# citiususc/BigSeqKit

Hardware: AMD Instinct MI355X
Metric: M records/s + GB/s (vs HBM roofline) on 100GB FASTQ stats (higher is better)
Workload: dtype u8; 1 GPU; bigseqkit stats on 100.0 GB synthetic FASTQ-150 (BASELINE C2: 315457413 records x 317 B), HBM-resident, 1 record-aligned shard(s); command=stats, records=315457413, bytes=99999999921, seed=42

## Files before the change

bigseqkit_amd/_lib.py:

```python
import ctypes as C
import os

_HERE = os.path.dirname(os.path.abspath(__file__))
LIB_PATH = os.environ.get("BSK_LIB", os.path.join(_HERE, "lib", "libbsk.so"))

if not os.path.exists(LIB_PATH):
    raise ImportError(
        f"libbsk.so not found at {LIB_PATH}: build it with ./build.sh "
        "(hipcc --offload-arch=gfx950); bigseqkit_amd has no CPU fallback")



def _preload_hip_runtime():
    import importlib.util
    try:
        spec = importlib.util.find_spec("torch")
    except Exception:
        spec = None
    if spec and spec.origin:
        cand = os.path.join(os.path.dirname(spec.origin), "lib", "libamdhip64.so")
        if os.path.exists(cand):
            try:
                C.CDLL(cand, mode=C.RTLD_GLOBAL)
            except OSError:
# ... 139 lines not shown
    "bsk_event_destroy": (_i, [_vp]),
    "bsk_selftest_regex_find": (_i, [C.c_char_p, C.c_char_p, _sz, _sz, _p(C.c_uint32), _p(C.c_uint32)]),
    "bsk_store_open": (_i, [C.c_char_p, _i, _p(_vp)]),
    "bsk_store_error": (C.c_char_p, [_vp]),
    "bsk_store_put": (_i, [_vp, _vp, _u64, _vp]),
    "bsk_store_put_host": (_i, [_vp, _u64, _vp, _sz]),
    "bsk_store_close": (_i, [_vp, _p(_u64)]),
    "bsk_run_to_store": (_i, [_vp, _vp, _sz, _i, _i64, _vp, _u64, _p(_u64), _p(_u64)]),
    "bsk_profile_enable": (_i, [_vp, _i]),
    "bsk_profile_read": (_i, [_vp, C.c_char_p, _p(C.c_double), _p(_u64)]),
    "bsk_profile_reset": (_i, [_vp]),
    "bsk_profile_dump": (_i, [_vp, C.c_char_p, _sz]),
    "bsk_selftest_scan": (_i, [_i, _p(C.c_uint32), _p(C.c_uint32)]),
    "bsk_selftest_rmdup_keys": (_i, [_vp, _p(_u64), _p(_u64), _sz, _p(_sz)]),
    "bsk_selftest_stream_read": (_i, [_vp, _sz, _i, _i, _p(C.c_float)]),
}

for _name, (_res, _args) in SIGNATURES.items():
    _f = getattr(lib, _name)
    _f.restype = _res
    _f.argtypes = _args


class BskError(RuntimeError):
    def __init__(self, code, message):
        super().__init__(message)
        self.code = code


def check(rc, ctx=None):
# ... 5 lines not shown
```

bigseqkit_amd/csrc/capi.cpp:

```cpp
#include <hip/hip_runtime_api.h>

#include <algorithm>
#include <cstdio>
#include <cstdlib>
#include <cstring>
#include <new>
#include <optional>

#include "../../include/bsk.h"
#include "anchor.hpp"
#include "ctx.hpp"
#include "ops_host.hpp"
#include "ops_host_internal.hpp"
#include "ops_segcopy.hpp"
#include "stats_host.hpp"
#include "stream_stats.hpp"
#include "regex_vm.hpp"
#include "synth.hpp"

namespace bsk {
hipError_t launch_synth(int kind, uint64_t seed, unsigned flags, uint64_t first_record, uint8_t* dst, uint64_t n,
                        hipStream_t st);
}

// ... 288 lines not shown
}

int bsk_rmdup_finish(bsk_ctx* c) {
    if (!c) return BSK_ERR_INVALID_ARG;
    if (c->op != bsk::Op::RmDup) return BSK_OK;
    return bsk::rmdup_finish(c);
}

void bsk_destroy(bsk_ctx* c) {
    if (!c) return;
    if (c->op == bsk::Op::RmDup) bsk::rmdup_finish(c);
    if (c->device >= 0) {
        hipSetDevice(c->device);
        hipDeviceSynchronize();
        for (auto& p : c->pending) { hipEventDestroy(p.a); hipEventDestroy(p.b); }
        bsk::store_drainer_free(c);
        if (c->d_anchors) hipFree(c->d_anchors);
        if (c->d_rng) hipFree(c->d_rng);
        if (c->d_parts) hipFree(c->d_parts);
        if (c->d_vec) hipFree(c->d_vec);
        if (c->d_pack) hipFree(c->d_pack);
        if (c->h_pack) hipHostFree(c->h_pack);
        if (c->d_ctl) hipFree(c->d_ctl);
        if (c->h_ctl) hipHostFree(c->h_ctl);
        if (c->h_head) hipHostFree(c->h_head);
        if (c->d_overflow) hipFree(c->d_overflow);
        for (void* p : {(void*)c->d_text_w, (void*)c->d_lin_off, (void*)c->d_lin, (void*)c->d_codon, (void*)c->d_keys,
                        (void*)c->d_table})
            if (p) hipFree(p);
        if (c->d_names) hipFree(c->d_names);
// ... 74 lines not shown
}

size_t bsk_stats_vector_len(const bsk_ctx* c) { return c ? (size_t)STATS_HDR + c->hist_cap : 0; }

int bsk_stats_reset(bsk_ctx* c, void* stream) {
    if (!c || c->op != Op::Stats) return fail(c, BSK_ERR_INVALID_ARG, "libbsk: not a Stats context");
    if (c->device < 0) return fail(c, BSK_ERR_NO_DEVICE, "libbsk: context was created without a device");
    BSK_ENTER(c);
    hipStream_t st = (hipStream_t)stream;
    HIP_TRY(c, hipMemsetAsync(c->d_vec, 0, ((size_t)STATS_HDR + c->hist_cap) * sizeof(uint64_t), st));
    HIP_TRY(c, hipMemsetAsync(c->d_ctl, 0, bsk_ctx::CTL_WORDS * sizeof(uint64_t), st));
    c->vec_reduced = false;
    return BSK_OK;
}

static int stats_run_device(bsk_ctx* c, const uint8_t* d_buf, size_t n, int format, uint64_t* d_vec, hipStream_t st) {
    const bool fastq = format == BSK_FORMAT_FASTQ;
    const bool all = c->opts.b("All");
    const bool variant = fastq ? c->stats_a_dense : c->tune.is("stats_fasta", "events");
    const int per_cu = stats_max_blocks_per_cu(fastq, all, c->use_dpp, variant);
    const int blocks = std::max(1, c->num_cus * per_cu);
    const uint64_t waves = (uint64_t)blocks * 4;
    const uint64_t nr = pick_nranges(n, waves, c->min_range_bytes, (int)c->tune.num("ranges_per_wave"));
    const uint32_t nranges = (uint32_t)nr;
    uint64_t chunk = (n + nranges - 1) / nranges;
    chunk = (chunk + 15) & ~(uint64_t)15;
    const bool self_anchor = fastq && !all && c->use_dpp && !c->tune.is("stats_prep", "pass");
    uint32_t tickets = nranges, nsplit = nranges;
    if (self_anchor) {
        chunk = (chunk + 63) & ~(uint64_t)63;
        const uint64_t tail = nranges / 16, small = chunk / 4;
        const uint64_t floor_bytes = std::max<uint64_t>(c->min_range_bytes, (uint64_t)c->tune.num("stats_tail", 192 << 10));
        if (tail && small >= floor_bytes && !c->tune.is("stats_tail", "uniform") && (uint64_t)(nranges - tail) * chunk < n) {
            nsplit = (uint32_t)(nranges - tail);
            tickets = nsplit + (uint32_t)((n - (uint64_t)nsplit * chunk + small - 1) / small);
        }
    } else {
        int rc = ensure_ranges(c, nranges);
        if (rc != BSK_OK) return rc;
    }
    const uint64_t need = n / c->hist_cap + 1024;
    if (need > c->overflow_cap) {
        uint64_t* nb = nullptr;
        HIP_TRY(c, hipMalloc((void**)&nb, need * sizeof(uint64_t)));
        if (c->d_overflow) {
            HIP_TRY(c, hipMemcpyAsync(nb, c->d_overflow, c->overflow_cap * sizeof(uint64_t), hipMemcpyDeviceToDevice, st));
            HIP_TRY(c, hipStreamSynchronize(st));
            HIP_TRY(c, hipFree(c->d_overflow));
        }
        c->d_overflow = nb;
        c->overflow_cap = need;
    }
// ... 34 lines not shown
            c->rng_cap = nranges;
        }
        D.r_head = c->d_rng;
        D.r_tail = c->d_rng + nranges;
        D.r_flags = reinterpret_cast<uint32_t*>(c->d_rng + 2 * (size_t)nranges);
        HIP_TRY(c, hipMemsetAsync(c->d_rng, 0, (size_t)nranges * 20, st));
    }
    if (!self_anchor) {
        Timed t(c, "k_prep", st);
        HIP_TRY(c, launch_prep(fastq, d_buf, n, chunk, nranges, anchors, queue, st, !fastq,
                               fastq ? nullptr : c->d_anchors + (size_t)nranges + 2));
    }
    {
        Timed t(c, "k_stats", st);
        HIP_TRY(c, launch_stats(fastq, all, c->use_dpp, blocks, d_buf, n, anchors, tickets, queue, D, st, variant,
                                !fastq ? chunk : 0, self_anchor ? chunk : 0, nsplit));
    }
    if (!fastq) HIP_TRY(c, launch_stats_stitch(nranges, D, st));
    if (all && (int)gap_letters.size() > MAX_GAP_LETTERS) {
        const int rci = build_index(c, d_buf, n, format, st);
        if (rci != BSK_OK) return rci;
        uint32_t set[8] = {0, 0, 0, 0, 0, 0, 0, 0};
        for (char ch : gap_letters) set[(uint8_t)ch >> 5] |= 1u << ((uint8_t)ch & 31u);
        HIP_TRY(c, launch_gap_set_count(d_buf, c->table, set, fastq, D.vec + 2, st));
    }
    return BSK_OK;
}

static int stage_shard(bsk_ctx* c, const void* shard, size_t n, int on_device, hipStream_t st, const uint8_t** d);

int bsk_stats_run(bsk_ctx* c, const void* shard, size_t n, int on_device, int format, int64_t pid, void* d_vec,
// ... 160 lines not shown
    c->type_if_F = alphabet_name(guess_alphabet_less_conservatively(seq.data(), seq.size(), 10000));
    *n_out = m.size();
    if (m.size() > cap || !keys || !vals) {
        if (cap == 0) return BSK_OK;
        return fail(c, BSK_ERR_CAPACITY, "libbsk: output map does not fit the caller's buffers");
    }
    size_t i = 0;
    for (auto& kv : m) {
        keys[i] = kv.first;
        vals[i] = kv.second;
        ++i;
    }
    return BSK_OK;
}

int bsk_stats_collect(bsk_ctx* c, const void* d_vec, int64_t* keys, int64_t* vals, size_t cap, size_t* n_out) {
    if (!c || c->op != Op::Stats) return fail(c, BSK_ERR_INVALID_ARG, "libbsk: not a Stats context");
    if (c->device < 0) return fail(c, BSK_ERR_NO_DEVICE, "libbsk: context was created without a device");
    if (!n_out) return fail(c, BSK_ERR_INVALID_ARG, "libbsk: null n_out");
    BSK_ENTER(c);
    HIP_TRY(c, hipDeviceSynchronize());
    const uint64_t* dv = d_vec ? (const uint64_t*)d_vec : c->d_vec;
    const uint32_t kbins = std::min<uint32_t>(bsk_ctx::PACK_BINS, c->hist_cap);
    const size_t pack_words = 8 + (size_t)STATS_HDR + kbins;
    if (!c->d_pack) HIP_TRY(c, hipMalloc((void**)&c->d_pack, pack_words * sizeof(uint64_t)));
    if (!c->h_pack) HIP_TRY(c, hipHostMalloc((void**)&c->h_pack, pack_words * sizeof(uint64_t), hipHostMallocDefault));
    HIP_TRY(c, launch_stats_pack(dv, c->hist_cap, c->d_status, c->d_pack, kbins, nullptr));
    HIP_TRY(c, hipMemcpyAsync(c->h_pack, c->d_pack, pack_words * sizeof(uint64_t), hipMemcpyDeviceToHost, nullptr));
    HIP_TRY(c, hipStreamSynchronize(nullptr));
    const uint64_t* status = c->h_pack;
    if (status[0]) {
        int code;
        std::string m = describe_kernel_errors(status[0], &code);
        return fail(c, code, m);
    }
    const size_t ext = (size_t)std::min<uint64_t>(status[2], c->hist_cap);
    const size_t len = (size_t)STATS_HDR + ext;
    std::vector<uint64_t> v(c->h_pack + 8, c->h_pack + 8 + std::min<size_t>(len, (size_t)STATS_HDR + kbins));
    if (ext > kbins) {
        v.resize(len);
        HIP_TRY(c, hipMemcpy(v.data() + STATS_HDR + kbins, dv + STATS_HDR + kbins, (ext - kbins) * sizeof(uint64_t), hipMemcpyDeviceToHost));
    }
    std::vector<uint64_t> ov;
    if (status[1]) {
// ... 603 lines not shown
    return BSK_OK;
}
int bsk_event_elapsed_ms(void* start, void* stop, float* ms) {
    HIP_TRY(nullptr, hipEventSynchronize((hipEvent_t)stop));
    HIP_TRY(nullptr, hipEventElapsedTime(ms, (hipEvent_t)start, (hipEvent_t)stop));
    return BSK_OK;
}
int bsk_event_destroy(void* ev) {
    HIP_TRY(nullptr, hipEventDestroy((hipEvent_t)ev));
    return BSK_OK;
}

int bsk_profile_enable(bsk_ctx* c, int on) {
    if (!c) return BSK_ERR_INVALID_ARG;
    c->profile = on != 0;
    return BSK_OK;
}

int bsk_profile_read(bsk_ctx* c, const char* kernel, double* total_ms, uint64_t* launches) {
    if (!c || !kernel) return BSK_ERR_INVALID_ARG;
    if (c->device >= 0) {
        BSK_ENTER(c);
        for (auto& p : c->pending) {
            HIP_TRY(c, hipEventSynchronize(p.b));
            float ms = 0;
            HIP_TRY(c, hipEventElapsedTime(&ms, p.a, p.b));
            auto& pr = c->prof[p.name];
            pr.ms += ms;
            pr.launches += 1;
            hipEventDestroy(p.a);
            hipEventDestroy(p.b);
        }
        c->pending.clear();
    }
    auto it = c->prof.find(kernel);
    if (total_ms) *total_ms = it == c->prof.end() ? 0.0 : it->second.ms;
    if (launches) *launches = it == c->prof.end() ? 0 : it->second.launches;
    return BSK_OK;
}

int bsk_profile_dump(bsk_ctx* c, char* buf, size_t cap) {
    if (!c || !buf || cap == 0) return BSK_ERR_INVALID_ARG;
    double d;
    uint64_t l;
    int rc = bsk_profile_read(c, "", &d, &l);
    if (rc != BSK_OK) return rc;
    std::string out;
// ... 49 lines not shown
        HIP_TRY(nullptr, hipEventRecord(a, nullptr));
        HIP_TRY(nullptr, launch_stream_read(blocks, (const uint8_t*)d_buf, n, chunk, (uint32_t)nr, d, d + 1, nullptr));
        HIP_TRY(nullptr, hipEventRecord(b, nullptr));
        HIP_TRY(nullptr, hipEventSynchronize(b));
        float ms = 0;
        HIP_TRY(nullptr, hipEventElapsedTime(&ms, a, b));
        if (r > 0) total += ms;
    }
    *avg_ms = total / reps;
    hipEventDestroy(a);
    hipEventDestroy(b);
    hipFree(d);
    return BSK_OK;
}

int bsk_selftest_scan(int use_dpp, const uint32_t* in64, uint32_t* out64) {
    uint32_t *d_in = nullptr, *d_out = nullptr;
    HIP_TRY(nullptr, hipMalloc((void**)&d_in, 64 * 4));
    HIP_TRY(nullptr, hipMalloc((void**)&d_out, 64 * 4));
    HIP_TRY(nullptr, hipMemcpy(d_in, in64, 64 * 4, hipMemcpyHostToDevice));
    HIP_TRY(nullptr, launch_scan_selftest(use_dpp != 0, d_in, d_out, nullptr));
    HIP_TRY(nullptr, hipMemcpy(out64, d_out, 64 * 4, hipMemcpyDeviceToHost));
    hipFree(d_in);
    hipFree(d_out);
    return BSK_OK;
}

int bsk_selftest_regex_find(const char* expr, const uint8_t* text, size_t n, size_t from, uint32_t* caps4, uint32_t* ngroups) {
    try {
        const VmProgram P = compile_vm(expr ? expr : "");
// ... 10 lines not shown
```

bigseqkit_amd/csrc/ctx.hpp:

```cpp
#pragma once
#include <hip/hip_runtime_api.h>

#include <algorithm>
#include <array>
#include <atomic>
#include <cstdlib>
#include <cctype>
#include <cstdint>
#include <cstdio>
#include <cstring>
#include <map>
#include <mutex>
#include <string>
#include <vector>

#include "index.hpp"
#include "opts.hpp"
#include "regex_nfa.hpp"
#include "regex_vm.hpp"

struct bsk_tuning {
    static const char* const* names() {
        static const char* const N[] = {"filter", "grep_shiftand", "head_genome_window", "index", "locate_nopre", "long_bytes", "min_range_bytes", "names",
                                        "names_scale", "out", "pin_alphabet", "ranges_per_wave", "replace", "rmdup", "rmdup_buckets", "rmdup_hash", "rmdup_k1_bits", "rmdup_k2_bits", "rmdup_keys", "rmdup_place", "rmdup_xcheck", "rmdup_xlocal", "scan", "segcopy",
                                        "sort", "stage_bytes", "stats_a", "stats_fasta", "stats_prep", "stats_tail", "subseq", "subseq_scale", "text", "translate", "translate_index", "translate_probe", "translate_stream", "tr_lanes", nullptr};
        return N;
    }
    std::map<std::string, std::string> v;
    static bool known(const std::string& k) {
        for (const char* const* n = names(); *n; ++n) if (k == *n) return true;
        return false;
    }
    void load_env() {
        for (const char* const* n = names(); *n; ++n) {
            std::string e = "BSK_";
            for (const char* q = *n; *q; ++q) e.push_back((char)toupper((unsigned char)*q));
            if (const char* val = getenv(e.c_str())) v[*n] = val;
        }
    }
    const char* get(const char* k) const {
// ... 250 lines not shown
    uint64_t slice_src_cap = 0;

    void* drainer = nullptr;
    uint8_t* pinned[2] = {nullptr, nullptr};
    uint8_t* d_stage[2] = {nullptr, nullptr};
    size_t stage_size[2] = {0, 0};
    hipStream_t copy_stream[2] = {nullptr, nullptr};
    hipEvent_t stage_done[2] = {nullptr, nullptr};
    hipEvent_t stage_free[2] = {nullptr, nullptr};

    bool profile = false;
    struct Prof { double ms = 0; uint64_t launches = 0; };
    std::map<std::string, Prof> prof;
    struct PendingEv { const char* name; hipEvent_t a, b; };
    std::vector<PendingEv> pending;

    void set_error(const std::string& m) const {
        std::lock_guard<std::mutex> g(mu);
        last_error = m;
    }

    mutable std::string log_text;
    void log(const char* level, const std::string& m, bool unless_quiet = false) const {
        if (unless_quiet && opts.cb("Quiet")) return;
        const std::string line = std::string("[") + level + "] " + m + "\n";
        {
            std::lock_guard<std::mutex> g(mu);
            log_text += line;
        }
        fputs(line.c_str(), stderr);
// ... 11 lines not shown
        if (owns) ++c->call_gen;
    }
    ~bsk_call_scope() { if (owns) c->busy.store(false, std::memory_order_release); }
    bsk_call_scope(const bsk_call_scope&) = delete;
    bsk_call_scope& operator=(const bsk_call_scope&) = delete;
};
#define BSK_BUSY_TEXT "libbsk: context busy: another call is running on this context (one context per caller thread, include/bsk.h)"

struct Timed {
    bsk_ctx* c;
    const char* name;
    hipStream_t st;
    hipEvent_t a = nullptr, b = nullptr;
    Timed(bsk_ctx* c_, const char* n, hipStream_t s) : c(c_), name(n), st(s) {
        if (c->profile) {
            hipEventCreate(&a);
            hipEventCreate(&b);
            hipEventRecord(a, st);
        }
    }
    ~Timed() {
        if (c->profile && a) {
            hipEventRecord(b, st);
            c->pending.push_back({name, a, b});
        }
    }
};

inline uint64_t pick_nranges(uint64_t n, uint64_t waves, uint64_t min_range_bytes, int pinned = 0) {
    uint64_t nr;
    if (pinned) nr = waves * (uint64_t)pinned;
    else {
        nr = n / (512u * 1024u);
        const uint64_t lo = std::min<uint64_t>(waves * 2, n / (128u * 1024u));
        nr = std::max(nr, lo);
        nr = std::min<uint64_t>(nr, waves * 16);
    }
    nr = std::min<uint64_t>(nr, n / std::max<uint64_t>(1, min_range_bytes));
    return std::max<uint64_t>(1, nr);
// ... 6 lines not shown
```

bigseqkit_amd/csrc/stream_stats.hip:

```cpp
#include <hip/hip_runtime.h>

#include <algorithm>
#include <cstdint>

#include "anchor.hpp"
#include "anchor_wave_dev.hpp"
#include "index.hpp"
#include "stream_core_dev.hpp"
#include "stream_fasta2_dev.hpp"
#include "stream_stats.hpp"

namespace bsk {

namespace {

using namespace stream;

constexpr int BIG_SLOTS = 64;
constexpr uint32_t BIG_EMPTY = 0xFFFFFFFFu;

__device__ __forceinline__ void add_big(uint32_t len, uint32_t c, uint32_t* s_hist, const StatsDev& D) {
    uint32_t* keys = s_hist + LDS_HIST;
    uint32_t* cnts = keys + BIG_SLOTS;
    const uint32_t slot = (len * 2654435761u) >> 26;
// ... 292 lines not shown
#define BSK_STATS_WAVES_FQ 6
#endif
#if BSK_STATS_WAVES
#ifndef BSK_STATS_WAVES_FA_ALL
#define BSK_STATS_WAVES_FA_ALL 5
#endif
#define BSK_STATS_ATTR __attribute__((amdgpu_waves_per_eu((ALL && FASTQ) ? BSK_STATS_WAVES_ALL : (FASTQ ? BSK_STATS_WAVES_FQ : ((ALL && ROLES_T) ? BSK_STATS_WAVES_FA_ALL : BSK_STATS_WAVES)), 8)))
#else
#define BSK_STATS_ATTR
#endif

template <bool FASTQ, bool ALL, bool DPP, bool ROLES_T = true>
__global__ __launch_bounds__(WAVES_PER_BLOCK * WAVE) BSK_STATS_ATTR void k_stats(const uint8_t* __restrict__ buf, uint64_t n,
                                                                   const uint64_t* __restrict__ anchors,
                                                                   uint32_t nranges, uint32_t* __restrict__ queue,
                                                                   StatsDev D, uint64_t chunk, uint32_t nsplit) {
    __shared__ uint32_t s_hist[LDS_HIST + 2 * BIG_SLOTS];
    constexpr bool ROLES = FASTQ && ALL && ROLES_T;
    constexpr bool SALL = ALL && !ROLES;
    constexpr int WINDOW = (FASTQ && !SALL) ? 256 : CAP;
    constexpr bool F2 = !FASTQ && ROLES_T;
    __shared__ Lds<FASTQ, SALL, F2 ? 4 : WINDOW> s_l[F2 ? 1 : WAVES_PER_BLOCK];
    __shared__ LdsF2T<F2 && ALL> s_f2[F2 ? WAVES_PER_BLOCK : 1];
    for (int i = threadIdx.x; i < LDS_HIST + 2 * BIG_SLOTS; i += blockDim.x)
        s_hist[i] = (i >= LDS_HIST && i < LDS_HIST + BIG_SLOTS) ? BIG_EMPTY : 0u;
    __syncthreads();

    const int lane = threadIdx.x & 63;
    const int wave = threadIdx.x >> 6;
    Lds<FASTQ, SALL, F2 ? 4 : WINDOW>& L = s_l[F2 ? 0 : wave];
    StatsSinkT<ROLES> sink;
    sink.s_hist = s_hist;
    sink.D = D;
    constexpr bool SELF = FASTQ && !ALL && DPP;
    const bool self_anchor = SELF && anchors == nullptr;
    const uint64_t n_eff = self_anchor ? wave_anchor::effective_end(buf, n) : anchors[nranges];
    uint64_t w20 = 0, w30 = 0, wgap = 0;
    for (;;) {
        uint32_t r = 0;
        if (lane == 0) r = atomicAdd(queue, 1u);
        r = wave_first(r);
        if (r >= nranges) break;
        uint64_t rs = 0, re = n_eff;
        if (self_anchor) {
            if constexpr (SELF) {
#pragma nounroll
                for (uint32_t k = 0; k < 2u; ++k) {
                    const uint32_t t = r + k;
                    if (t == 0u || t >= nranges) continue;
                    const uint64_t from = t <= nsplit ? (uint64_t)t * chunk : (uint64_t)nsplit * chunk + (uint64_t)(t - nsplit) * (chunk >> 2);
                    uint32_t flo = (uint32_t)from, fhi = (uint32_t)(from >> 32);
                    asm volatile("" : "+v"(flo), "+v"(fhi));
                    const uint64_t av = wave_anchor::fastq_range_start(buf, n, ((uint64_t)fhi << 32) | flo);
                    const uint64_t a = ((uint64_t)wave_first((uint32_t)(av >> 32)) << 32) | wave_first((uint32_t)av);
                    if (k == 0u) rs = a;
                    else re = a;
                }
            }
        } else {
            rs = anchors[r];
            re = anchors[r + 1];
        }
        rs = rs < n_eff ? rs : n_eff;
// ... 168 lines not shown
        const uint64_t rs = (uint64_t)r * chunk, re = (rs + chunk < n) ? rs + chunk : n;
        for (uint64_t t = rs; t < re; t += TILE) {
#pragma unroll
            for (int p = 0; p < NPIECE; ++p) {
                const uint64_t idx = t + (uint64_t)p * PIECE_BYTES + (uint64_t)lane * 16;
                if (idx + 16 <= re) {
                    const uint4 v = *reinterpret_cast<const uint4*>(buf + idx);
                    acc ^= v.x ^ v.y ^ v.z ^ v.w;
                }
            }
        }
    }
    if (acc == 0x9E3779B9u) sink[0] = acc;
}

template <bool DPP>
__global__ void k_scan_selftest(const uint32_t* in, uint32_t* out) {
    out[threadIdx.x] = wave_incl_scan<DPP>(in[threadIdx.x]);
}

}

hipError_t launch_prep(bool fastq, const uint8_t* buf, uint64_t n, uint64_t chunk, uint32_t nranges,
                       uint64_t* anchors, uint32_t* queue, hipStream_t st, bool line_mode, uint64_t* raw) {
    const int threads = 256;
    const int blocks = (int)(((uint64_t)nranges + 1 + 3) / 4);
    if (fastq) hipLaunchKernelGGL(k_prep<true>, dim3(blocks), dim3(threads), 0, st, buf, n, chunk, nranges, anchors, queue, 0);
    else if (line_mode && raw) {
        hipLaunchKernelGGL(k_prep<false>, dim3(blocks), dim3(threads), 0, st, buf, n, chunk, nranges, raw, queue, 2);
        hipLaunchKernelGGL(k_prep_fill, dim3((nranges + 1 + 255) / 256), dim3(256), 0, st, (const uint64_t*)raw, nranges, anchors);
    } else hipLaunchKernelGGL(k_prep<false>, dim3(blocks), dim3(threads), 0, st, buf, n, chunk, nranges, anchors, queue, line_mode ? 1 : 0);
    return hipGetLastError();
}

__global__ __launch_bounds__(1024) void k_stats_pack(const uint64_t* __restrict__ vec, uint32_t cap, const uint64_t* __restrict__ status,
                                                     uint64_t* __restrict__ pack, uint32_t kbins) {
    __shared__ uint32_t s_hi;
    if (threadIdx.x == 0) s_hi = 0;
    __syncthreads();
    const uint64_t* hist = vec + STATS_HDR;
    uint32_t hi = 0;
    for (uint32_t base = threadIdx.x; base < cap; base += 8u * 1024u) {
        uint64_t h[8];
#pragma unroll
        for (uint32_t k = 0; k < 8u; ++k) {
            const uint32_t i = base + k * 1024u;
            h[k] = i < cap ? hist[i] : 0ull;
        }
#pragma unroll
        for (uint32_t k = 0; k < 8u; ++k)
            if (h[k]) hi = base + k * 1024u + 1u;
    }
    if (hi) atomicMax(&s_hi, hi);
    for (uint32_t i = threadIdx.x; i < (uint32_t)STATS_HDR + kbins; i += 1024u) pack[8u + i] = vec[i];
    if (threadIdx.x < 8u && threadIdx.x != 2u) pack[threadIdx.x] = status[threadIdx.x];
    __syncthreads();
    if (threadIdx.x == 0) pack[2] = s_hi;
}

hipError_t launch_stats_pack(const uint64_t* vec, uint32_t cap, const uint64_t* status, uint64_t* pack, uint32_t kbins, hipStream_t st) {
    if (kbins > cap) kbins = cap;
    hipLaunchKernelGGL(k_stats_pack, dim3(1), dim3(1024), 0, st, vec, cap, status, pack, kbins);
    return hipGetLastError();
}

namespace {
struct GapSet { uint32_t w[8]; };
__global__ __launch_bounds__(256) void k_gap_set_count(const uint8_t* __restrict__ buf, RecordTable t, GapSet S, int fastq,
                                                       unsigned long long* __restrict__ gap_slot) {
    const uint32_t lane = threadIdx.x & 63u;
    const uint64_t nwaves = (uint64_t)gridDim.x * (blockDim.x >> 6);
    uint64_t acc = 0;
    for (uint64_t r = (uint64_t)blockIdx.x * (blockDim.x >> 6) + (threadIdx.x >> 6); r < t.n; r += nwaves) {
        const uint64_t from = t.start[r] + t.l_head[r] + 1;
        const uint64_t to = fastq ? from + t.l_seq[r] : t.start[r + 1];
        for (uint64_t i = from + lane; i < to; i += 64) {
            const uint8_t c = buf[i];
// ... 10 lines not shown
    if (t.n == 0) return hipSuccess;
    GapSet S;
    for (int i = 0; i < 8; ++i) S.w[i] = set[i];
    const uint64_t blocks = std::min<uint64_t>((t.n + 3) / 4, 256ull * 32ull);
    hipLaunchKernelGGL(k_gap_set_count, dim3((unsigned)blocks), dim3(256), 0, st, buf, t, S, fastq ? 1 : 0, (unsigned long long*)gap_slot);
    return hipGetLastError();
}

hipError_t launch_stats_stitch(uint32_t nranges, const StatsDev& D, hipStream_t st) {
    hipLaunchKernelGGL(k_stats_stitch, dim3((nranges + 255u) / 256u), dim3(256), 0, st, nranges, D);
    return hipGetLastError();
}

template <bool FASTQ, bool ALL, bool ROLES_T = true>
static hipError_t launch_stats_t(bool dpp, int blocks, const uint8_t* buf, uint64_t n, const uint64_t* anchors,
                                 uint32_t nranges, uint32_t* queue, const StatsDev& D, hipStream_t st, uint64_t chunk, uint32_t nsplit = 0) {
    const dim3 b(WAVES_PER_BLOCK * WAVE);
    if (dpp) hipLaunchKernelGGL((k_stats<FASTQ, ALL, true, ROLES_T>), dim3(blocks), b, 0, st, buf, n, anchors, nranges, queue, D, chunk, nsplit);
    else hipLaunchKernelGGL((k_stats<FASTQ, ALL, false, ROLES_T>), dim3(blocks), b, 0, st, buf, n, anchors, nranges, queue, D, chunk, nsplit);
    return hipGetLastError();
}

hipError_t launch_stats(bool fastq, bool all, bool dpp, int blocks, const uint8_t* buf, uint64_t n,
                        const uint64_t* anchors, uint32_t nranges, uint32_t* queue, const StatsDev& D,
                        hipStream_t st, bool a_dense, uint64_t skip_chunk, uint64_t fq_chunk, uint32_t fq_nsplit) {
    if (fastq && all && a_dense) return launch_stats_t<true, true, false>(dpp, blocks, buf, n, anchors, nranges, queue, D, st, fq_chunk, fq_nsplit);
    if (fastq) return all ? launch_stats_t<true, true>(dpp, blocks, buf, n, anchors, nranges, queue, D, st, fq_chunk, fq_nsplit)
                          : launch_stats_t<true, false>(dpp, blocks, buf, n, anchors, nranges, queue, D, st, fq_chunk, fq_nsplit);
    if (all) return a_dense ? launch_stats_t<false, true, false>(dpp, blocks, buf, n, anchors, nranges, queue, D, st, skip_chunk)
                            : launch_stats_t<false, true>(dpp, blocks, buf, n, anchors, nranges, queue, D, st, skip_chunk);
    return a_dense ? launch_stats_t<false, false, false>(dpp, blocks, buf, n, anchors, nranges, queue, D, st, skip_chunk)
                   : launch_stats_t<false, false>(dpp, blocks, buf, n, anchors, nranges, queue, D, st, skip_chunk);
}

int stats_max_blocks_per_cu(bool fastq, bool all, bool dpp, bool a_dense) {
    int nb = 0;
    const void* f = nullptr;
#define BSK_PICK(FQ, AL, RO)                                                             \
    f = dpp ? (const void*)k_stats<FQ, AL, true, RO> : (const void*)k_stats<FQ, AL, false, RO>;
    if (fastq && all && a_dense) { BSK_PICK(true, true, false) }
    else if (fastq && all) { BSK_PICK(true, true, true) }
    else if (fastq) { BSK_PICK(true, false, true) }
    else if (all && a_dense) { BSK_PICK(false, true, false) }
    else if (all) { BSK_PICK(false, true, true) }
    else if (a_dense) { BSK_PICK(false, false, false) }
    else { BSK_PICK(false, false, true) }
#undef BSK_PICK
    if (hipOccupancyMaxActiveBlocksPerMultiprocessor(&nb, f, WAVES_PER_BLOCK * WAVE, 0) != hipSuccess || nb < 1) nb = 1;
    return nb;
}

hipError_t launch_stream_read(int blocks, const uint8_t* buf, uint64_t n, uint64_t chunk, uint32_t nranges,
                              uint32_t* queue, uint32_t* sink, hipStream_t st) {
    hipLaunchKernelGGL(k_stream_read, dim3(blocks), dim3(WAVES_PER_BLOCK * WAVE), 0, st, buf, n, chunk, nranges, queue,
                       sink);
    return hipGetLastError();
}

hipError_t launch_scan_selftest(bool dpp, const uint32_t* in, uint32_t* out, hipStream_t st) {
    if (dpp) hipLaunchKernelGGL(k_scan_selftest<true>, dim3(1), dim3(64), 0, st, in, out);
    else hipLaunchKernelGGL(k_scan_selftest<false>, dim3(1), dim3(64), 0, st, in, out);
    return hipGetLastError();
}

}
```

bigseqkit_amd/csrc/stream_stats.hpp:

```cpp
#pragma once
#include <hip/hip_runtime_api.h>

#include <cstdint>

namespace bsk {

constexpr int STATS_HDR = 8;
constexpr int MAX_GAP_LETTERS = 8;

constexpr uint32_t ERR_BAD_HEADER = 1u;
constexpr uint32_t ERR_BAD_PLUS = 2u;
constexpr uint32_t ERR_LEN_MISMATCH = 4u;
constexpr uint32_t ERR_TRUNCATED = 8u;
constexpr uint32_t ERR_ANCHOR = 16u;
constexpr uint32_t ERR_LINE_TOO_LONG = 32u;
constexpr uint32_t ERR_CAPACITY = 64u;

struct PredConsts {
    uint32_t k20, k30;
    uint32_t gap_rep[MAX_GAP_LETTERS];
    int ngap;
    uint32_t kgap;
};

// ... 6 lines not shown
    PredConsts pred;
    uint64_t* r_head;
    uint64_t* r_tail;
    uint32_t* r_flags;
};

constexpr uint32_t RF_VISITED = 1u, RF_HAS_HEADER = 2u, RF_HEAD_CLOSED = 4u, RF_TAIL_OPEN = 8u;
constexpr uint32_t RF_MID = 16u, RF_SKIP_SEQ = 32u;

hipError_t launch_prep(bool fastq, const uint8_t* buf, uint64_t n, uint64_t chunk, uint32_t nranges,
                       uint64_t* anchors, uint32_t* queue, hipStream_t st, bool line_mode = false, uint64_t* raw = nullptr);
hipError_t launch_stats_stitch(uint32_t nranges, const StatsDev& D, hipStream_t st);
struct RecordTable;
hipError_t launch_gap_set_count(const uint8_t* buf, const RecordTable& t, const uint32_t (&set)[8], bool fastq, uint64_t* gap_slot,
                                hipStream_t st);
hipError_t launch_stats_pack(const uint64_t* vec, uint32_t cap, const uint64_t* status, uint64_t* pack, uint32_t kbins, hipStream_t st);
hipError_t launch_stats(bool fastq, bool all, bool dpp, int blocks, const uint8_t* buf, uint64_t n,
                        const uint64_t* anchors, uint32_t nranges, uint32_t* queue, const StatsDev& D,
                        hipStream_t st, bool a_dense = false, uint64_t skip_chunk = 0,
                        uint64_t fq_chunk = 0, uint32_t fq_nsplit = 0);
int stats_max_blocks_per_cu(bool fastq, bool all, bool dpp, bool a_dense = false);
hipError_t launch_stream_read(int blocks, const uint8_t* buf, uint64_t n, uint64_t chunk, uint32_t nranges,
                              uint32_t* queue, uint32_t* sink, hipStream_t st);
hipError_t launch_scan_selftest(bool dpp, const uint32_t* in, uint32_t* out, hipStream_t st);

}
```

include/bsk.h:

```cpp
#ifndef BSK_H
#define BSK_H

#include <stddef.h>
#include <stdint.h>

#ifdef __cplusplus
extern "C" {
#endif

#define BSK_OK 0
#define BSK_ERR_INVALID_ARG 1
#define BSK_ERR_OPTS 2
#define BSK_ERR_FORMAT 3
#define BSK_ERR_UNSUPPORTED 4
#define BSK_ERR_HIP 5
#define BSK_ERR_NO_DEVICE 6
#define BSK_ERR_CAPACITY 7
#define BSK_ERR_OVERFLOW_EXCHANGE 8

#define BSK_FORMAT_FASTA 0
#define BSK_FORMAT_FASTQ 1

typedef struct bsk_ctx bsk_ctx;

// ... 194 lines not shown
int bsk_synth_device(int kind, uint64_t seed, unsigned flags, uint64_t first_record, void* d_dst, size_t n, int device,
                     void* stream);

int bsk_event_create(void** ev);
int bsk_event_record(void* ev, void* stream);
int bsk_event_elapsed_ms(void* start, void* stop, float* ms);
int bsk_event_destroy(void* ev);
int bsk_profile_enable(bsk_ctx* ctx, int on);
int bsk_profile_read(bsk_ctx* ctx, const char* kernel, double* total_ms, uint64_t* launches);
int bsk_profile_reset(bsk_ctx* ctx);
int bsk_profile_dump(bsk_ctx* ctx, char* buf, size_t cap);

int bsk_selftest_scan(int use_dpp, const uint32_t* in64, uint32_t* out64);
int bsk_selftest_rmdup_keys(bsk_ctx* ctx, uint64_t* k1, uint64_t* k2, size_t cap, size_t* n_out);
int bsk_selftest_stream_read(const void* d_buf, size_t n, int reps, int blocks_per_cu, float* avg_ms);

#ifdef __cplusplus
}
#endif
#endif
```

Measured before the change: 20960 M records/s.

## Add ticket runs to stats, parallel multi-block pack, event pooling, NT read probe

Factors ticket and range planning into a helper and adds an optional 'stats_run' knob that lets each wave claim several consecutive body ranges per ticket. It defaults to 1, which keeps the old behaviour. The single-block stats pack kernel is replaced by a 32-block version that reduces through a scratch counter, aiming to cut final pack latency. Profiling events are pooled instead of being created and destroyed for every launch. A new streaming-read selftest and a pack selftest are added. The multi-block pack adds atomic, last-block coordination that could misbehave if the scratch word is left dirty.

Result: no change. 20980 M records/s, median of 4 (+0.1%).

```diff
diff --git a/bigseqkit_amd/_lib.py b/bigseqkit_amd/_lib.py
--- a/bigseqkit_amd/_lib.py
+++ b/bigseqkit_amd/_lib.py
@@ -177,6 +177,8 @@
     "bsk_selftest_scan": (_i, [_i, _p(C.c_uint32), _p(C.c_uint32)]),
     "bsk_selftest_rmdup_keys": (_i, [_vp, _p(_u64), _p(_u64), _sz, _p(_sz)]),
     "bsk_selftest_stream_read": (_i, [_vp, _sz, _i, _i, _p(C.c_float)]),
+    "bsk_selftest_stream_read_nt": (_i, [_vp, _sz, _i, _p(C.c_float)]),
+    "bsk_selftest_stats_pack": (_i, [_vp, _vp, _p(_u64), _sz, _p(_sz)]),
 }
 
 for _name, (_res, _args) in SIGNATURES.items():
diff --git a/bigseqkit_amd/csrc/capi.cpp b/bigseqkit_amd/csrc/capi.cpp
--- a/bigseqkit_amd/csrc/capi.cpp
+++ b/bigseqkit_amd/csrc/capi.cpp
@@ -326,6 +326,7 @@
         hipSetDevice(c->device);
         hipDeviceSynchronize();
         for (auto& p : c->pending) { hipEventDestroy(p.a); hipEventDestroy(p.b); }
+        for (hipEvent_t e : c->ev_pool) hipEventDestroy(e);
         bsk::store_drainer_free(c);
         if (c->d_anchors) hipFree(c->d_anchors);
         if (c->d_rng) hipFree(c->d_rng);
@@ -430,6 +431,31 @@
     return BSK_OK;
 }
 
+struct StatsTickets { uint32_t nranges, tickets, nsplit, run; uint64_t chunk; };
+static StatsTickets stats_tickets(const bsk_ctx* c, uint64_t n, uint64_t waves, bool self_anchor) {
+    const uint64_t min_range = c ? c->min_range_bytes : (uint64_t)MIN_RANGE_BYTES;
+    auto tune_num = [&](const char* k, long long dflt) { return c ? c->tune.num(k, dflt) : dflt; };
+    StatsTickets T;
+    T.nranges = (uint32_t)pick_nranges(n, waves, min_range, (int)tune_num("ranges_per_wave", 0));
+    T.chunk = (n + T.nranges - 1) / T.nranges;
+    T.chunk = (T.chunk + 15) & ~(uint64_t)15;
+    T.tickets = T.nsplit = T.nranges;
+    T.run = 1;
+    if (!self_anchor) return T;
+    T.chunk = (T.chunk + 63) & ~(uint64_t)63;
+    const uint64_t tail = T.nranges / 16, small = T.chunk / 4;
+    const uint64_t floor_bytes = std::max<uint64_t>(min_range, (uint64_t)tune_num("stats_tail", 192 << 10));
+    if (tail && small >= floor_bytes && !(c && c->tune.is("stats_tail", "uniform")) && (uint64_t)(T.nranges - tail) * T.chunk < n) {
+        T.nsplit = (uint32_t)(T.nranges - tail);
+        T.tickets = T.nsplit + (uint32_t)((n - (uint64_t)T.nsplit * T.chunk + small - 1) / small);
+    }
+    const long long pinned = tune_num("stats_run", 0);
+    uint64_t run = pinned > 0 ? (uint64_t)pinned : 1u;
+    run = std::min<uint64_t>(run, std::max<uint64_t>(1, (1ull << 30) / std::max<uint64_t>(1, T.chunk)));
+    T.run = (uint32_t)std::min<uint64_t>(run, 1u << 16);
+    return T;
+}
+
 static int stats_run_device(bsk_ctx* c, const uint8_t* d_buf, size_t n, int format, uint64_t* d_vec, hipStream_t st) {
     const bool fastq = format == BSK_FORMAT_FASTQ;
     const bool all = c->opts.b("All");
@@ -437,21 +463,11 @@
     const int per_cu = stats_max_blocks_per_cu(fastq, all, c->use_dpp, variant);
     const int blocks = std::max(1, c->num_cus * per_cu);
     const uint64_t waves = (uint64_t)blocks * 4;
-    const uint64_t nr = pick_nranges(n, waves, c->min_range_bytes, (int)c->tune.num("ranges_per_wave"));
-    const uint32_t nranges = (uint32_t)nr;
-    uint64_t chunk = (n + nranges - 1) / nranges;
-    chunk = (chunk + 15) & ~(uint64_t)15;
     const bool self_anchor = fastq && !all && c->use_dpp && !c->tune.is("stats_prep", "pass");
-    uint32_t tickets = nranges, nsplit = nranges;
-    if (self_anchor) {
-        chunk = (chunk + 63) & ~(uint64_t)63;
-        const uint64_t tail = nranges / 16, small = chunk / 4;
-        const uint64_t floor_bytes = std::max<uint64_t>(c->min_range_bytes, (uint64_t)c->tune.num("stats_tail", 192 << 10));
-        if (tail && small >= floor_bytes && !c->tune.is("stats_tail", "uniform") && (uint64_t)(nranges - tail) * chunk < n) {
-            nsplit = (uint32_t)(nranges - tail);
-            tickets = nsplit + (uint32_t)((n - (uint64_t)nsplit * chunk + small - 1) / small);
-        }
-    } else {
+    const StatsTickets T = stats_tickets(c, n, waves, self_anchor);
+    const uint32_t nranges = T.nranges, tickets = T.tickets, nsplit = T.nsplit, run = T.run;
+    const uint64_t chunk = T.chunk;
+    if (!self_anchor) {
         int rc = ensure_ranges(c, nranges);
         if (rc != BSK_OK) return rc;
     }
@@ -516,7 +532,7 @@
     {
         Timed t(c, "k_stats", st);
         HIP_TRY(c, launch_stats(fastq, all, c->use_dpp, blocks, d_buf, n, anchors, tickets, queue, D, st, variant,
-                                !fastq ? chunk : 0, self_anchor ? chunk : 0, nsplit));
+                                !fastq ? chunk : 0, self_anchor ? chunk : 0, nsplit, run));
     }
     if (!fastq) HIP_TRY(c, launch_stats_stitch(nranges, D, st));
     if (all && (int)gap_letters.size() > MAX_GAP_LETTERS) {
@@ -707,6 +723,33 @@
     return BSK_OK;
 }
 
+static int stats_pack_to_host(bsk_ctx* c, const uint64_t* dv) {
+    const uint32_t kbins = std::min<uint32_t>(bsk_ctx::PACK_BINS, c->hist_cap);
+    const size_t pack_words = 8 + (size_t)STATS_HDR + kbins;
+    if (!c->d_pack) {
+        HIP_TRY(c, hipMalloc((void**)&c->d_pack, (pack_words + 1) * sizeof(uint64_t)));
+        HIP_TRY(c, hipMemset(c->d_pack + pack_words, 0, sizeof(uint64_t)));
+    }
+    if (!c->h_pack) HIP_TRY(c, hipHostMalloc((void**)&c->h_pack, pack_words * sizeof(uint64_t), hipHostMallocDefault));
+    HIP_TRY(c, launch_stats_pack(dv, c->hist_cap, c->d_status, c->d_pack, kbins, reinterpret_cast<uint32_t*>(c->d_pack + pack_words), nullptr));
+    HIP_TRY(c, hipMemcpyAsync(c->h_pack, c->d_pack, pack_words * sizeof(uint64_t), hipMemcpyDeviceToHost, nullptr));
+    HIP_TRY(c, hipStreamSynchronize(nullptr));
+    return BSK_OK;
+}
+
+int bsk_selftest_stats_pack(bsk_ctx* c, const void* d_vec, uint64_t* pack, size_t cap_words, size_t* n_words) {
+    if (!c || c->op != Op::Stats || !n_words) return fail(c, BSK_ERR_INVALID_ARG, "libbsk: bad argument");
+    if (c->device < 0) return fail(c, BSK_ERR_NO_DEVICE, "libbsk: context was created without a device");
+    BSK_ENTER(c);
+    HIP_TRY(c, hipDeviceSynchronize());
+    *n_words = 8 + (size_t)STATS_HDR + std::min<uint32_t>(bsk_ctx::PACK_BINS, c->hist_cap);
+    if (!pack || cap_words < *n_words) return fail(c, BSK_ERR_CAPACITY, "libbsk: packet does not fit the caller's buffer");
+    int rc = stats_pack_to_host(c, d_vec ? (const uint64_t*)d_vec : c->d_vec);
+    if (rc != BSK_OK) return rc;
+    memcpy(pack, c->h_pack, *n_words * sizeof(uint64_t));
+    return BSK_OK;
+}
+
 int bsk_stats_collect(bsk_ctx* c, const void* d_vec, int64_t* keys, int64_t* vals, size_t cap, size_t* n_out) {
     if (!c || c->op != Op::Stats) return fail(c, BSK_ERR_INVALID_ARG, "libbsk: not a Stats context");
     if (c->device < 0) return fail(c, BSK_ERR_NO_DEVICE, "libbsk: context was created without a device");
@@ -715,12 +758,8 @@
     HIP_TRY(c, hipDeviceSynchronize());
     const uint64_t* dv = d_vec ? (const uint64_t*)d_vec : c->d_vec;
     const uint32_t kbins = std::min<uint32_t>(bsk_ctx::PACK_BINS, c->hist_cap);
-    const size_t pack_words = 8 + (size_t)STATS_HDR + kbins;
-    if (!c->d_pack) HIP_TRY(c, hipMalloc((void**)&c->d_pack, pack_words * sizeof(uint64_t)));
-    if (!c->h_pack) HIP_TRY(c, hipHostMalloc((void**)&c->h_pack, pack_words * sizeof(uint64_t), hipHostMallocDefault));
-    HIP_TRY(c, launch_stats_pack(dv, c->hist_cap, c->d_status, c->d_pack, kbins, nullptr));
-    HIP_TRY(c, hipMemcpyAsync(c->h_pack, c->d_pack, pack_words * sizeof(uint64_t), hipMemcpyDeviceToHost, nullptr));
-    HIP_TRY(c, hipStreamSynchronize(nullptr));
+    int rcp = stats_pack_to_host(c, dv);
+    if (rcp != BSK_OK) return rcp;
     const uint64_t* status = c->h_pack;
     if (status[0]) {
         int code;
@@ -1354,6 +1393,14 @@
 int bsk_profile_enable(bsk_ctx* c, int on) {
     if (!c) return BSK_ERR_INVALID_ARG;
     c->profile = on != 0;
+    if (on && c->device >= 0) {
+        BSK_ENTER(c);
+        while (c->ev_pool.size() < bsk_ctx::EV_POOL_FILL) {
+            hipEvent_t e = nullptr;
+            HIP_TRY(c, hipEventCreate(&e));
+            c->ev_pool.push_back(e);
+        }
+    }
     return BSK_OK;
 }
 
@@ -1368,9 +1415,8 @@
             auto& pr = c->prof[p.name];
             pr.ms += ms;
             pr.launches += 1;
-            hipEventDestroy(p.a);
-            hipEventDestroy(p.b);
         }
+        for (auto& p : c->pending) { c->ev_pool.push_back(p.a); c->ev_pool.push_back(p.b); }
         c->pending.clear();
     }
     auto it = c->prof.find(kernel);
@@ -1450,6 +1496,37 @@
     return BSK_OK;
 }
 
+int bsk_selftest_stream_read_nt(const void* d_buf, size_t n, int reps, float* avg_ms) {
+    if (!d_buf || !avg_ms || reps < 1 || n == 0) return fail_global(BSK_ERR_INVALID_ARG, "libbsk: bad argument");
+    int dev = 0;
+    HIP_TRY(nullptr, hipGetDevice(&dev));
+    hipDeviceProp_t p;
+    HIP_TRY(nullptr, hipGetDeviceProperties(&p, dev));
+    const int blocks = std::max(1, p.multiProcessorCount * stats_max_blocks_per_cu(true, false, true));
+    const StatsTickets T = stats_tickets(nullptr, n, (uint64_t)blocks * 4, true);
+    uint32_t* d = nullptr;
+    HIP_TRY(nullptr, hipMalloc((void**)&d, 8));
+    hipEvent_t a, b;
+    HIP_TRY(nullptr, hipEventCreate(&a));
+    HIP_TRY(nullptr, hipEventCreate(&b));
+    float total = 0;
+    for (int r = 0; r < reps + 1; ++r) {
+        HIP_TRY(nullptr, hipMemsetAsync(d, 0, 8, nullptr));
+        HIP_TRY(nullptr, hipEventRecord(a, nullptr));
+        HIP_TRY(nullptr, launch_stream_read_nt(blocks, (const uint8_t*)d_buf, n, T.chunk, T.tickets, T.nsplit, d, d + 1, nullptr));
+        HIP_TRY(nullptr, hipEventRecord(b, nullptr));
+        HIP_TRY(nullptr, hipEventSynchronize(b));
+        float ms = 0;
+        HIP_TRY(nullptr, hipEventElapsedTime(&ms, a, b));
+        if (r > 0) total += ms;
+    }
+    *avg_ms = total / reps;
+    hipEventDestroy(a);
+    hipEventDestroy(b);
+    hipFree(d);
+    return BSK_OK;
+}
+
 int bsk_selftest_scan(int use_dpp, const uint32_t* in64, uint32_t* out64) {
     uint32_t *d_in = nullptr, *d_out = nullptr;
     HIP_TRY(nullptr, hipMalloc((void**)&d_in, 64 * 4));
diff --git a/bigseqkit_amd/csrc/ctx.hpp b/bigseqkit_amd/csrc/ctx.hpp
--- a/bigseqkit_amd/csrc/ctx.hpp
+++ b/bigseqkit_amd/csrc/ctx.hpp
@@ -23,7 +23,7 @@
     static const char* const* names() {
         static const char* const N[] = {"filter", "grep_shiftand", "head_genome_window", "index", "locate_nopre", "long_bytes", "min_range_bytes", "names",
                                         "names_scale", "out", "pin_alphabet", "ranges_per_wave", "replace", "rmdup", "rmdup_buckets", "rmdup_hash", "rmdup_k1_bits", "rmdup_k2_bits", "rmdup_keys", "rmdup_place", "rmdup_xcheck", "rmdup_xlocal", "scan", "segcopy",
-                                        "sort", "stage_bytes", "stats_a", "stats_fasta", "stats_prep", "stats_tail", "subseq", "subseq_scale", "text", "translate", "translate_index", "translate_probe", "translate_stream", "tr_lanes", nullptr};
+                                        "sort", "stage_bytes", "stats_a", "stats_fasta", "stats_prep", "stats_run", "stats_tail", "subseq", "subseq_scale", "text", "translate", "translate_index", "translate_probe", "translate_stream", "tr_lanes", nullptr};
         return N;
     }
     std::map<std::string, std::string> v;
@@ -304,6 +304,14 @@
     std::map<std::string, Prof> prof;
     struct PendingEv { const char* name; hipEvent_t a, b; };
     std::vector<PendingEv> pending;
+    std::vector<hipEvent_t> ev_pool;
+    static constexpr size_t EV_POOL_FILL = 64;
+    hipEvent_t ev_take() {
+        hipEvent_t e = nullptr;
+        if (!ev_pool.empty()) { e = ev_pool.back(); ev_pool.pop_back(); }
+        else if (hipEventCreate(&e) != hipSuccess) e = nullptr;
+        return e;
+    }
 
     void set_error(const std::string& m) const {
         std::lock_guard<std::mutex> g(mu);
@@ -345,15 +353,18 @@
     hipEvent_t a = nullptr, b = nullptr;
     Timed(bsk_ctx* c_, const char* n, hipStream_t s) : c(c_), name(n), st(s) {
         if (c->profile) {
-            hipEventCreate(&a);
-            hipEventCreate(&b);
-            hipEventRecord(a, st);
+            a = c->ev_take();
+            b = c->ev_take();
+            if (a) hipEventRecord(a, st);
         }
     }
     ~Timed() {
-        if (c->profile && a) {
+        if (c->profile && a && b) {
             hipEventRecord(b, st);
             c->pending.push_back({name, a, b});
+        } else {
+            if (a) c->ev_pool.push_back(a);
+            if (b) c->ev_pool.push_back(b);
         }
     }
 };
diff --git a/bigseqkit_amd/csrc/stream_stats.hip b/bigseqkit_amd/csrc/stream_stats.hip
--- a/bigseqkit_amd/csrc/stream_stats.hip
+++ b/bigseqkit_amd/csrc/stream_stats.hip
@@ -330,7 +330,7 @@
 __global__ __launch_bounds__(WAVES_PER_BLOCK * WAVE) BSK_STATS_ATTR void k_stats(const uint8_t* __restrict__ buf, uint64_t n,
                                                                    const uint64_t* __restrict__ anchors,
                                                                    uint32_t nranges, uint32_t* __restrict__ queue,
-                                                                   StatsDev D, uint64_t chunk, uint32_t nsplit) {
+                                                                   StatsDev D, uint64_t chunk, uint32_t nsplit, uint32_t run) {
     __shared__ uint32_t s_hist[LDS_HIST + 2 * BIG_SLOTS];
     constexpr bool ROLES = FASTQ && ALL && ROLES_T;
     constexpr bool SALL = ALL && !ROLES;
@@ -340,6 +340,15 @@
     __shared__ LdsF2T<F2 && ALL> s_f2[F2 ? WAVES_PER_BLOCK : 1];
     for (int i = threadIdx.x; i < LDS_HIST + 2 * BIG_SLOTS; i += blockDim.x)
         s_hist[i] = (i >= LDS_HIST && i < LDS_HIST + BIG_SLOTS) ? BIG_EMPTY : 0u;
+    __shared__ uint32_t s_plan[FASTQ && !ALL && DPP ? 3 : 1];
+    if constexpr (FASTQ && !ALL && DPP) {
+        if (threadIdx.x == 0) {
+            const uint32_t pb = run > 1u ? (nsplit + run - 1u) / run : nsplit;
+            s_plan[0] = run;
+            s_plan[1] = pb;
+            s_plan[2] = pb + (nranges - nsplit);
+        }
+    }
     __syncthreads();
 
     const int lane = threadIdx.x & 63;
@@ -356,13 +365,26 @@
         uint32_t r = 0;
         if (lane == 0) r = atomicAdd(queue, 1u);
         r = wave_first(r);
-        if (r >= nranges) break;
+        uint32_t r_end = r + 1u;
+        if (SELF && self_anchor) {
+            const uint32_t p_run = wave_first(s_plan[0]), p_body = wave_first(s_plan[1]), p_draws = wave_first(s_plan[2]);
+            if (r >= p_draws) break;
+            if (p_run > 1u) {
+                if (r < p_body) {
+                    r *= p_run;
+                    r_end = r + p_run < nsplit ? r + p_run : nsplit;
+                } else {
+                    r = nsplit + (r - p_body);
+                    r_end = r + 1u;
+                }
+            }
+        } else if (r >= nranges) break;
         uint64_t rs = 0, re = n_eff;
         if (self_anchor) {
             if constexpr (SELF) {
 #pragma nounroll
                 for (uint32_t k = 0; k < 2u; ++k) {
-                    const uint32_t t = r + k;
+                    const uint32_t t = k ? r_end : r;
                     if (t == 0u || t >= nranges) continue;
                     const uint64_t from = t <= nsplit ? (uint64_t)t * chunk : (uint64_t)nsplit * chunk + (uint64_t)(t - nsplit) * (chunk >> 2);
                     uint32_t flo = (uint32_t)from, fhi = (uint32_t)(from >> 32);
@@ -561,6 +583,39 @@
     if (acc == 0x9E3779B9u) sink[0] = acc;
 }
 
+__global__ __launch_bounds__(WAVES_PER_BLOCK * WAVE) void k_stream_read_nt(const uint8_t* __restrict__ buf, uint64_t n,
+                                                                            uint64_t chunk, uint32_t nranges, uint32_t nsplit,
+                                                                            uint32_t* __restrict__ queue,
+                                                                            uint32_t* __restrict__ sink) {
+    const int lane = threadIdx.x & 63;
+    uint32_t acc = 0;
+    for (;;) {
+        uint32_t r = 0;
+        if (lane == 0) r = atomicAdd(queue, 1u);
+        r = wave_first(r);
+        if (r >= nranges) break;
+        uint64_t rs = 0, re = n;
+#pragma unroll
+        for (uint32_t k = 0; k < 2u; ++k) {
+            const uint32_t t = r + k;
+            if (t == 0u || t >= nranges) continue;
+            const uint64_t from = t <= nsplit ? (uint64_t)t * chunk : (uint64_t)nsplit * chunk + (uint64_t)(t - nsplit) * (chunk >> 2);
+            if (k == 0u) rs = from;
+            else re = from;
+        }
+        rs = rs < n ? rs : n;
+        re = re < n ? re : n;
+        if (rs >= re) continue;
+        for (uint64_t tile_idx = tile_grid_start(buf, rs); tile_idx < re; tile_idx += TILE) {
+            uint4 cur[NPIECE];
+            load_tile<true>(cur, buf, n, rs, re, tile_idx);
+#pragma unroll
+            for (int p = 0; p < NPIECE; ++p) acc ^= cur[p].x ^ cur[p].y ^ cur[p].z ^ cur[p].w;
+        }
+    }
+    if (acc == 0x9E3779B9u) sink[0] = acc;
+}
+
 template <bool DPP>
 __global__ void k_scan_selftest(const uint32_t* in, uint32_t* out) {
     out[threadIdx.x] = wave_incl_scan<DPP>(in[threadIdx.x]);
@@ -580,34 +635,49 @@
     return hipGetLastError();
 }
 
-__global__ __launch_bounds__(1024) void k_stats_pack(const uint64_t* __restrict__ vec, uint32_t cap, const uint64_t* __restrict__ status,
-                                                     uint64_t* __restrict__ pack, uint32_t kbins) {
+constexpr uint32_t PACK_BLOCKS = 32, PACK_THREADS = 256;
+__global__ __launch_bounds__(PACK_THREADS) void k_stats_pack(const uint64_t* __restrict__ vec, uint32_t cap, const uint64_t* __restrict__ status,
+                                                             uint64_t* __restrict__ pack, uint32_t kbins, uint32_t* __restrict__ scratch) {
     __shared__ uint32_t s_hi;
     if (threadIdx.x == 0) s_hi = 0;
     __syncthreads();
     const uint64_t* hist = vec + STATS_HDR;
+    const uint32_t slice = (cap + gridDim.x - 1u) / gridDim.x;
+    const uint32_t lo = blockIdx.x * slice < cap ? blockIdx.x * slice : cap, end = cap - lo < slice ? cap : lo + slice;
     uint32_t hi = 0;
-    for (uint32_t base = threadIdx.x; base < cap; base += 8u * 1024u) {
+    for (uint32_t base = lo + threadIdx.x; base < end; base += 8u * PACK_THREADS) {
         uint64_t h[8];
 #pragma unroll
         for (uint32_t k = 0; k < 8u; ++k) {
-            const uint32_t i = base + k * 1024u;
-            h[k] = i < cap ? hist[i] : 0ull;
+            const uint32_t i = base + k * PACK_THREADS;
+            h[k] = i < end ? hist[i] : 0ull;
         }
 #pragma unroll
         for (uint32_t k = 0; k < 8u; ++k)
-            if (h[k]) hi = base + k * 1024u + 1u;
+            if (h[k]) hi = base + k * PACK_THREADS + 1u;
     }
     if (hi) atomicMax(&s_hi, hi);
-    for (uint32_t i = threadIdx.x; i < (uint32_t)STATS_HDR + kbins; i += 1024u) pack[8u + i] = vec[i];
-    if (threadIdx.x < 8u && threadIdx.x != 2u) pack[threadIdx.x] = status[threadIdx.x];
+    for (uint32_t i = blockIdx.x * PACK_THREADS + threadIdx.x; i < (uint32_t)STATS_HDR + kbins; i += gridDim.x * PACK_THREADS) pack[8u + i] = vec[i];
     __syncthreads();
-    if (threadIdx.x == 0) pack[2] = s_hi;
-}
-
-hipError_t launch_stats_pack(const uint64_t* vec, uint32_t cap, const uint64_t* status, uint64_t* pack, uint32_t kbins, hipStream_t st) {
+    if (threadIdx.x == 0) {
+        if (s_hi) atomicMax(scratch, s_hi);
+        __threadfence();
+        const uint32_t before = atomicAdd(scratch + 1, 1u);
+        __threadfence();
+        if (before == gridDim.x - 1u) {
+            pack[2] = atomicExch(scratch, 0u);
+            atomicExch(scratch + 1, 0u);
+#pragma unroll
+            for (uint32_t k = 0; k < 8u; ++k)
+                if (k != 2u) pack[k] = status[k];
+        }
+    }
+}
+
+hipError_t launch_stats_pack(const uint64_t* vec, uint32_t cap, const uint64_t* status, uint64_t* pack, uint32_t kbins, uint32_t* scratch,
+                             hipStream_t st) {
     if (kbins > cap) kbins = cap;
-    hipLaunchKernelGGL(k_stats_pack, dim3(1), dim3(1024), 0, st, vec, cap, status, pack, kbins);
+    hipLaunchKernelGGL(k_stats_pack, dim3(PACK_BLOCKS), dim3(PACK_THREADS), 0, st, vec, cap, status, pack, kbins, scratch);
     return hipGetLastError();
 }
 
@@ -648,19 +718,19 @@
 
 template <bool FASTQ, bool ALL, bool ROLES_T = true>
 static hipError_t launch_stats_t(bool dpp, int blocks, const uint8_t* buf, uint64_t n, const uint64_t* anchors,
-                                 uint32_t nranges, uint32_t* queue, const StatsDev& D, hipStream_t st, uint64_t chunk, uint32_t nsplit = 0) {
+                                 uint32_t nranges, uint32_t* queue, const StatsDev& D, hipStream_t st, uint64_t chunk, uint32_t nsplit = 0, uint32_t run = 1) {
     const dim3 b(WAVES_PER_BLOCK * WAVE);
-    if (dpp) hipLaunchKernelGGL((k_stats<FASTQ, ALL, true, ROLES_T>), dim3(blocks), b, 0, st, buf, n, anchors, nranges, queue, D, chunk, nsplit);
-    else hipLaunchKernelGGL((k_stats<FASTQ, ALL, false, ROLES_T>), dim3(blocks), b, 0, st, buf, n, anchors, nranges, queue, D, chunk, nsplit);
+    if (dpp) hipLaunchKernelGGL((k_stats<FASTQ, ALL, true, ROLES_T>), dim3(blocks), b, 0, st, buf, n, anchors, nranges, queue, D, chunk, nsplit, run);
+    else hipLaunchKernelGGL((k_stats<FASTQ, ALL, false, ROLES_T>), dim3(blocks), b, 0, st, buf, n, anchors, nranges, queue, D, chunk, nsplit, run);
     return hipGetLastError();
 }
 
 hipError_t launch_stats(bool fastq, bool all, bool dpp, int blocks, const uint8_t* buf, uint64_t n,
                         const uint64_t* anchors, uint32_t nranges, uint32_t* queue, const StatsDev& D,
-                        hipStream_t st, bool a_dense, uint64_t skip_chunk, uint64_t fq_chunk, uint32_t fq_nsplit) {
+                        hipStream_t st, bool a_dense, uint64_t skip_chunk, uint64_t fq_chunk, uint32_t fq_nsplit, uint32_t fq_run) {
     if (fastq && all && a_dense) return launch_stats_t<true, true, false>(dpp, blocks, buf, n, anchors, nranges, queue, D, st, fq_chunk, fq_nsplit);
     if (fastq) return all ? launch_stats_t<true, true>(dpp, blocks, buf, n, anchors, nranges, queue, D, st, fq_chunk, fq_nsplit)
-                          : launch_stats_t<true, false>(dpp, blocks, buf, n, anchors, nranges, queue, D, st, fq_chunk, fq_nsplit);
+                          : launch_stats_t<true, false>(dpp, blocks, buf, n, anchors, nranges, queue, D, st, fq_chunk, fq_nsplit, fq_run ? fq_run : 1u);
     if (all) return a_dense ? launch_stats_t<false, true, false>(dpp, blocks, buf, n, anchors, nranges, queue, D, st, skip_chunk)
                             : launch_stats_t<false, true>(dpp, blocks, buf, n, anchors, nranges, queue, D, st, skip_chunk);
     return a_dense ? launch_stats_t<false, false, false>(dpp, blocks, buf, n, anchors, nranges, queue, D, st, skip_chunk)
@@ -691,6 +761,13 @@
     return hipGetLastError();
 }
 
+hipError_t launch_stream_read_nt(int blocks, const uint8_t* buf, uint64_t n, uint64_t chunk, uint32_t nranges, uint32_t nsplit,
+                                 uint32_t* queue, uint32_t* sink, hipStream_t st) {
+    hipLaunchKernelGGL(k_stream_read_nt, dim3(blocks), dim3(WAVES_PER_BLOCK * WAVE), 0, st, buf, n, chunk, nranges, nsplit, queue,
+                       sink);
+    return hipGetLastError();
+}
+
 hipError_t launch_scan_selftest(bool dpp, const uint32_t* in, uint32_t* out, hipStream_t st) {
     if (dpp) hipLaunchKernelGGL(k_scan_selftest<true>, dim3(1), dim3(64), 0, st, in, out);
     else hipLaunchKernelGGL(k_scan_selftest<false>, dim3(1), dim3(64), 0, st, in, out);
diff --git a/bigseqkit_amd/csrc/stream_stats.hpp b/bigseqkit_amd/csrc/stream_stats.hpp
--- a/bigseqkit_amd/csrc/stream_stats.hpp
+++ b/bigseqkit_amd/csrc/stream_stats.hpp
@@ -44,14 +44,17 @@
 struct RecordTable;
 hipError_t launch_gap_set_count(const uint8_t* buf, const RecordTable& t, const uint32_t (&set)[8], bool fastq, uint64_t* gap_slot,
                                 hipStream_t st);
-hipError_t launch_stats_pack(const uint64_t* vec, uint32_t cap, const uint64_t* status, uint64_t* pack, uint32_t kbins, hipStream_t st);
+hipError_t launch_stats_pack(const uint64_t* vec, uint32_t cap, const uint64_t* status, uint64_t* pack, uint32_t kbins, uint32_t* scratch,
+                             hipStream_t st);
 hipError_t launch_stats(bool fastq, bool all, bool dpp, int blocks, const uint8_t* buf, uint64_t n,
                         const uint64_t* anchors, uint32_t nranges, uint32_t* queue, const StatsDev& D,
                         hipStream_t st, bool a_dense = false, uint64_t skip_chunk = 0,
-                        uint64_t fq_chunk = 0, uint32_t fq_nsplit = 0);
+                        uint64_t fq_chunk = 0, uint32_t fq_nsplit = 0, uint32_t fq_run = 1);
 int stats_max_blocks_per_cu(bool fastq, bool all, bool dpp, bool a_dense = false);
 hipError_t launch_stream_read(int blocks, const uint8_t* buf, uint64_t n, uint64_t chunk, uint32_t nranges,
                               uint32_t* queue, uint32_t* sink, hipStream_t st);
+hipError_t launch_stream_read_nt(int blocks, const uint8_t* buf, uint64_t n, uint64_t chunk, uint32_t nranges, uint32_t nsplit,
+                                 uint32_t* queue, uint32_t* sink, hipStream_t st);
 hipError_t launch_scan_selftest(bool dpp, const uint32_t* in, uint32_t* out, hipStream_t st);
 
 }
diff --git a/include/bsk.h b/include/bsk.h
--- a/include/bsk.h
+++ b/include/bsk.h
@@ -232,6 +232,8 @@
 int bsk_selftest_scan(int use_dpp, const uint32_t* in64, uint32_t* out64);
 int bsk_selftest_rmdup_keys(bsk_ctx* ctx, uint64_t* k1, uint64_t* k2, size_t cap, size_t* n_out);
 int bsk_selftest_stream_read(const void* d_buf, size_t n, int reps, int blocks_per_cu, float* avg_ms);
+int bsk_selftest_stream_read_nt(const void* d_buf, size_t n, int reps, float* avg_ms);
+int bsk_selftest_stats_pack(bsk_ctx* ctx, const void* d_vec, uint64_t* pack, size_t cap_words, size_t* n_words);
 
 #ifdef __cplusplus
 }
```
